# MoZhou1995/DeepPDE_ActorCritic

Measured on AMD Instinct MI355X. Metric: SDE trajectory-steps/sec (batch×horizon) at d=20; value-fn rel-L2 vs analytic, higher is better.
Workload: dtype f32

## Files before the change

### deeppde_actorcritic_amd/csrc/dpac_rollout_staged.h

```cpp
#pragma once

#ifndef DPAC_ST_CHUNKS
#define DPAC_ST_CHUNKS 4
#endif
#ifndef DPAC_ST_TIGHT
#define DPAC_ST_TIGHT 0
#endif
#ifndef DPAC_ST_TIGHT_CHUNKS
#define DPAC_ST_TIGHT_CHUNKS 3
#endif
#ifndef DPAC_ST_PREFETCH
#define DPAC_ST_PREFETCH 1
#endif
constexpr int kStCW = 4;
constexpr int kStCH = 16;
constexpr int kStPrefetch = DPAC_ST_PREFETCH;
static_assert(kStPrefetch == 0 || kStPrefetch == 1, "DPAC_ST_PREFETCH is 0 or 1");
template <typename T, int D, int P>
struct StagedPlan {
  static constexpr int TPW = kStCW * (64 / P);
  static constexpr int SLOT = TPW * D * (int)sizeof(T);
  static constexpr int PIECES = (SLOT + 1023) / 1024;
  static constexpr int kLdsCap = 128 * 1024;
  static constexpr int SLOT_1K = (SLOT + 16 + 1023) / 1024 * 1024;
  static constexpr int SLOT_16 = (SLOT + 16 + 15) / 16 * 16;
  static constexpr bool kWide = !DPAC_ST_TIGHT && DPAC_ST_CHUNKS * kStCH * SLOT_1K <= kLdsCap;
  static constexpr int CHUNKS = kWide ? DPAC_ST_CHUNKS : DPAC_ST_TIGHT_CHUNKS;
  static constexpr int SLOT_LDS = kWide ? SLOT_1K : SLOT_16;
  static constexpr int PADOFF = SLOT_LDS - 16;
  static constexpr int RS = CHUNKS * kStCH;
  static_assert(P < 4 || (SLOT % 16 == 0 && (PIECES - 1) * 1024 + 16 <= SLOT), "DMA pieces stay inside the slot");
  static constexpr bool kOk = P >= 4 && RS * SLOT_LDS <= kLdsCap && kStCH * PIECES <= 62;
};

template <class Fn, int... S>
__device__ __forceinline__ void unroll_phases(Fn& fn, std::integer_sequence<int, S...>) {
  (fn(Phase<S>{}), ...);
}

__device__ __forceinline__ int lds_load_relaxed(const int* p) {
  return __hip_atomic_load(p, __ATOMIC_RELAXED, __HIP_MEMORY_SCOPE_WORKGROUP);
}
__device__ __forceinline__ void lds_store_relaxed(int* p, int v) {
  __hip_atomic_store(p, v, __ATOMIC_RELAXED, __HIP_MEMORY_SCOPE_WORKGROUP);
}

template <int GEN>
constexpr int st_waves() { return kStCW + (GEN > 0 ? GEN : 1); }
#ifndef DPAC_ST_GEN
#define DPAC_ST_GEN 12
#endif
constexpr int kStGen = DPAC_ST_GEN;
static_assert(64 * st_waves<kStGen>() <= 1024, "DPAC_ST_GEN: a workgroup holds at most 1024 threads");

__device__ __forceinline__ void st_wait_consumed(const int* s_done, int need) {
  for (;;) {
    int mn = lds_load_relaxed(&s_done[0]);
#pragma unroll
    for (int w = 1; w < kStCW; ++w) mn = min(mn, lds_load_relaxed(&s_done[w]));
    if (mn >= need) break;
    __builtin_amdgcn_s_sleep(2);
  }
}
template <int NREADY>
__device__ __forceinline__ void st_wait_published(const int* s_ready, int want) {
  for (;;) {
    int mn = lds_load_relaxed(&s_ready[0]);
#pragma unroll
    for (int w = 1; w < NREADY; ++w) mn = min(mn, lds_load_relaxed(&s_ready[w]));
    if (mn >= want) break;
    __builtin_amdgcn_s_sleep(1);
  }
}

#ifndef DPAC_ST_TRACE
#define DPAC_ST_TRACE 0
#endif
#if DPAC_ST_TRACE
constexpr int kStTraceRow = 128, kStTraceWaves = 16, kStTraceChunks = 32;
static __device__ uint32_t g_st_trace[2 * kStTraceWaves * kStTraceRow];
__device__ __forceinline__ uint32_t st_clock() {
  unsigned long long t;
  __builtin_amdgcn_sched_barrier(0);
  asm volatile("s_memtime %0\n\ts_waitcnt lgkmcnt(0)" : "=s"(t)::"memory");
  __builtin_amdgcn_sched_barrier(0);
  return (uint32_t)t;
}
__device__ __forceinline__ uint32_t st_realtime() {
  unsigned long long t;
  __builtin_amdgcn_sched_barrier(0);
  asm volatile("s_memrealtime %0\n\ts_waitcnt lgkmcnt(0)" : "=s"(t)::"memory");
  __builtin_amdgcn_sched_barrier(0);
  return (uint32_t)t;
}
#define ST_PUT(pt, v)                \
  do {                               \
    const uint32_t st_v_ = (v);      \
    if (st_on) st_row[(pt)] = st_v_; \
  } while (0)
#define ST_MARK(pt) ST_PUT(pt, st_clock())
#define ST_CHUNK(base, c0) ((base) + ((c0) / kStCH < kStTraceChunks ? (c0) / kStCH : kStTraceChunks - 1))
#else
#define ST_PUT(pt, v) \
  do {                \
  } while (0)
#define ST_MARK(pt) \
  do {              \
  } while (0)
#endif

template <typename T, class E, int D, int SCHEME, int OUT, int GEN = 0>
__global__ __launch_bounds__(64 * st_waves<GEN>()) void k_rollout_staged(const E eq, const DevConsts<T> c,
                                                                          const RolloutArgs<T> a) {
  constexpr int P = E::kP, M = E::M, MC = E::MC;
  using PL = StagedPlan<T, D, P>;
  constexpr int TPW = PL::TPW, RS = PL::RS, PIECES = PL::PIECES, SLOT_LDS = PL::SLOT_LDS;
  constexpr bool COST = (OUT & kOutCost) != 0, WANT_U = (OUT & kOutU) != 0;
  constexpr int F = P < kStCH ? P : kStCH;
  constexpr int NREADY = GEN > 0 ? GEN : 1;
  static_assert(kStCH % F == 0 && (F & (F - 1)) == 0, "flush phase fixed per unrolled body");
  static_assert(GEN == 0 || (2 * M <= 4 && kStCH % 2 == 0), "generators draw the paired layout");
  using TR = Transition<T, E, SCHEME>;
  __shared__ __attribute__((aligned(16))) unsigned char s_ring[RS * SLOT_LDS];
  __shared__ int s_ready[NREADY], s_done[kStCW];
  const int wave = __builtin_amdgcn_readfirstlane((int)threadIdx.x / 64), lane = (int)threadIdx.x % 64;
  const int64_t row0 = xcd_block(blockIdx.x, gridDim.x) * TPW;
  const int N = a.N;
#if DPAC_ST_TRACE
  const bool st_on = lane == 0 && wave < kStTraceWaves && (blockIdx.x == 0 || blockIdx.x == gridDim.x - 1);
  uint32_t* const st_row = g_st_trace + ((blockIdx.x == 0 ? 0 : kStTraceWaves) + (wave < kStTraceWaves ? wave : 0)) * kStTraceRow;
  ST_MARK(0);
  ST_PUT(5, st_realtime());
#endif
  if (threadIdx.x == 0) {
#pragma unroll
    for (int w = 0; w < NREADY; ++w) s_ready[w] = 0;
#pragma unroll
    for (int w = 0; w < kStCW; ++w) s_done[w] = 0;
  }
  if (threadIdx.x < RS * 4)
    reinterpret_cast<uint32_t*>(s_ring + (threadIdx.x / 4) * SLOT_LDS + PL::PADOFF)[threadIdx.x % 4] = 0u;
  __syncthreads();
  ST_MARK(1);

  if constexpr (GEN > 0) {
    if (wave >= kStCW) {
      const int g = wave - kStCW;
      const int64_t rows_live = (a.B - row0) < TPW ? (a.B - row0) : TPW;
      constexpr int PLS = (D + M - 1) / M;
      constexpr int NBLK = (kStCH / 2) * TPW * PLS;
      constexpr int PASSES = (NBLK + 64 * GEN - 1) / (64 * GEN);
      constexpr int SLOT_T = SLOT_LDS / (int)sizeof(T);
      T* const ringw = reinterpret_cast<T*>(s_ring);
      for (int c0 = 0; c0 < N; c0 += kStCH) {
        const int need = c0 + kStCH - RS;
        if (need > 0) st_wait_consumed(s_done, need);
        asm volatile("" ::: "memory");
#pragma unroll 1
        for (int k = 0; k < PASSES; ++k) {
          const int e = (k * GEN + g) * 64 + lane;
          const int u = e / (TPW * PLS), rem = e - u * (TPW * PLS);
          const int i = rem / PLS, p = rem - i * PLS;
          const int t0 = c0 + 2 * u;
          if (e < NBLK && t0 < N && i < rows_live) {
            T v[4];
            dw_block_values<T>(a.seed, (uint64_t)(a.traj_offset + row0 + i), (uint64_t)(t0 >> 1) * P + p,
                               a.sample_type, v);
            T* d0 = ringw + (t0 % RS) * SLOT_T + i * D + p * M;
            T* d1 = ringw + ((t0 + 1) % RS) * SLOT_T + i * D + p * M;
#pragma unroll
            for (int m = 0; m < M; ++m) {
              if (p * M + m < D) {
                d0[m] = v[m];
                if (t0 + 1 < N) d1[m] = v[M + m];
              }
            }
          }
        }
        asm volatile("s_waitcnt lgkmcnt(0)" ::: "memory");
        if (lane == 0) lds_store_relaxed(&s_ready[g], c0 + kStCH < N ? c0 + kStCH : N);
      }
      return;
    }
  } else if (wave == kStCW) {
    const int64_t rows_live = (a.B - row0) < TPW ? (a.B - row0) : TPW;
    const uint32_t bytes = (uint32_t)(rows_live * D * (int64_t)sizeof(T));
    const uint32_t lds0 = (uint32_t)(uintptr_t)(__attribute__((address_space(3))) unsigned char*)s_ring;
    const char* base = (const char*)(a.dw + row0 * D);
    const int64_t step_bytes = a.B * D * (int64_t)sizeof(T);
    for (int c0 = 0; c0 < N; c0 += kStCH) {
      const int need = c0 + kStCH - RS;
      if (need > 0) st_wait_consumed(s_done, need);
      asm volatile("" ::: "memory");
#if DPAC_ST_TRACE
      ST_MARK(ST_CHUNK(16, c0));
#endif
#pragma unroll
      for (int s = 0; s < kStCH; ++s) {
        const int t = c0 + s < N ? c0 + s : N - 1;
        const char* src = base + t * step_bytes;
        const uint32_t slot = lds0 + (uint32_t)((t % RS) * SLOT_LDS);
#pragma unroll
        for (int k = 0; k < PIECES; ++k) {
          const uint32_t off = (uint32_t)((k * 64 + lane) * 16);
          const char* gp = src + (off < bytes ? off : 0u);
          const uint32_t m0 = __builtin_amdgcn_readfirstlane(slot + (uint32_t)(k * 1024));
          if (off < bytes || lane == 0) {
            int keep;
            asm volatile("s_mov_b32 %0, m0\n\ts_mov_b32 m0, %2\n\ts_nop 0\n\tglobal_load_lds_dwordx4 %1, off\n\ts_mov_b32 m0, %0"
                         : "=&s"(keep) : "v"(gp), "s"(m0) : "memory");
          }
        }
      }
#if DPAC_ST_TRACE
      ST_MARK(ST_CHUNK(48, c0));
#endif
      if (c0 > 0) {
        asm volatile("s_waitcnt vmcnt(%0)" ::"n"(kStCH * PIECES) : "memory");
        if (lane == 0) lds_store_relaxed(&s_ready[0], c0);
#if DPAC_ST_TRACE
        ST_MARK(ST_CHUNK(80, c0));
#endif
      }
    }
    asm volatile("s_waitcnt vmcnt(0)" ::: "memory");
    if (lane == 0) lds_store_relaxed(&s_ready[0], N);
    ST_MARK(4);
    ST_PUT(6, st_realtime());
    return;
  }

  const LaneCoord<P> lc(a.B, lane, row0 + wave * (64 / P));
  const int gl = wave * (64 / P) + lane / P;
  const Own<D, P> own(lc.p);
  const Own<E::CDIM, P> ownu(lc.p);
  const BufSlab<T, D, P> sx(own, lc.b, lc.live);
  const BufSlab<T, E::CDIM, P> su(ownu, lc.b, lc.live);
  const uint32_t slab = (uint32_t)(a.B * D * sizeof(T));
  const uint32_t slab_u = (uint32_t)(a.B * E::CDIM * sizeof(T));
  const uint32_t row_bytes = (uint32_t)(N * sizeof(T));
  const __amdgpu_buffer_rsrc_t rs_x = make_rsrc(a.x, slab * (uint32_t)(N + 1));
  const __amdgpu_buffer_rsrc_t rs_u = make_rsrc(a.u, WANT_U ? slab_u * (uint32_t)N : 0u);
  const __amdgpu_buffer_rsrc_t rs_dt = make_rsrc(a.dt, (uint32_t)a.B * row_bytes);
  const __amdgpu_buffer_rsrc_t rs_cf = make_rsrc(a.coef, (uint32_t)a.B * row_bytes);
  const T* ring = reinterpret_cast<const T*>(s_ring);
  const int lds_e = gl * D + lc.p * M;
  constexpr bool kVecRead = Own<D, P>::kFull && (M * sizeof(T) == 8 || M * sizeof(T) == 16);
  const uint32_t lane_off = own.active() ? (uint32_t)(lds_e * (int)sizeof(T)) : (uint32_t)PL::PADOFF;
  T keep = 0;
  auto flush = [&](int t_last, int count) {
    const uint32_t off = (lc.live && lc.p < count)
                             ? (uint32_t)((lc.b * N + t_last - lc.p) * (int64_t)sizeof(T)) : kOOB;
    buf_store_scalar<T>(rs_dt, off, fabs(keep));
    buf_store_scalar<T>(rs_cf, off, keep > T(0) ? T(1) : T(0));
  };
  T x[M];
  sx.load(make_rsrc(a.x0, slab), x);
  sx.store(rs_x, x);
  T r = TR::kRadius ? dsqrt(Lanes<P>::sum(sumsq(x))) : T(0);
  Flags fl = SCHEME == DPAC_SCHEME_ADAPTIVE ? region(r, c) : Flags{true, false};
  T disc = 1, y = 0;
  T xc[M], rc = r;
#pragma unroll
  for (int m = 0; m < M; ++m) xc[m] = x[m];
  T Ra = fl.alive ? c.R : -std::numeric_limits<T>::infinity();
  bool alive = fl.alive;
  const T sq0 = SCHEME == DPAC_SCHEME_ADAPTIVE ? dsqrt(c.dt0) : c.sqrt_dt0;
  T dt = c.dt0, sq = sq0;
  if constexpr (SCHEME == DPAC_SCHEME_ADAPTIVE) {
    dt = adaptive_dt_raw(fl.layer, r, c);
    dt = fl.layer ? fmax(dt, c.dt_min) : dt;
    sq = dsqrt(dt);
  }
  ST_MARK(2);
  auto read_dw_at = [&](int t, uint32_t slot_bytes, T (&dwv)[M]) {
    if constexpr (kVecRead) {
      typedef T vec __attribute__((ext_vector_type(M)));
      const vec v = *reinterpret_cast<const vec*>(s_ring + slot_bytes + lane_off);
#pragma unroll
      for (int m = 0; m < M; ++m) dwv[m] = v[m];
    } else {
      const T* slot = ring + (t % RS) * (SLOT_LDS / (int)sizeof(T)) + lds_e;
#pragma unroll
      for (int m = 0; m < M; ++m) dwv[m] = own.valid(m) ? slot[m] : T(0);
    }
  };
  auto read_dw = [&](int t, T (&dwv)[M]) { read_dw_at(t, (uint32_t)((t % RS) * SLOT_LDS), dwv); };
  auto step = [&](int t, const T (&dwv)[M], auto phase) {
    T uc[MC], f[M], s[M], xt[M];
    eq.u_true(xc, rc, uc);
    eq.drift(xc, uc, rc, f);
    eq.sigma(xc, uc, s);
#pragma unroll
    for (int m = 0; m < M; ++m) xt[m] = xc[m] + fma(f[m], dt, (s[m] * dwv[m]) * sq);
    const T St = Lanes<P>::sum(sumsq(xt));
    T u[MC];
    if constexpr (COST || WANT_U) eq.u_true(x, r, u);
    bool coef;
    T rt = T(0), dtn = dt, sqn = sq;
    if constexpr (SCHEME == DPAC_SCHEME_ADAPTIVE) {
      rt = dsqrt(St);
      const T b = Ra - rt;
      const bool inner = b - c.c_layer > T(0);
      coef = b > T(0);
      const T dtb = fmax((b * b) * c.inv_den, c.dt_min);
      const T sqb = dsqrt(dtb);
      const bool layer = coef && !inner;
      dtn = layer ? dtb : c.dt0;
      sqn = layer ? sqb : sq0;
      Ra = coef ? Ra : -std::numeric_limits<T>::infinity();
    } else {
      if constexpr (E::kNeedsNorm) rt = dsqrt(St);
      coef = alive && !(St - c.R2 >= T(0));
      alive = coef;
    }
    if constexpr (COST) {
      const T cf = coef ? T(1) : T(0);
      const T w = eq.w_finish(Lanes<P>::sum(eq.w_part(x, u)));
      y += cost_increment(a.cost_order, w, cf, dt, disc);
      disc = disc * disc_factor(dt, cf, c);
    }
    const T kv = coef ? dt : -dt;
#pragma unroll
    for (int m = 0; m < M; ++m) {
      x[m] = coef ? xt[m] : x[m];
      xc[m] = xt[m];
    }
    if constexpr (E::kNeedsNorm) {
      r = coef ? rt : r;
      rc = rt;
    }
    dt = dtn;
    sq = sqn;
    sx.template store<DPAC_ROLLOUT_X_AUX>(rs_x, x, (uint32_t)(t + 1) * slab);
    if constexpr (WANT_U) su.store(rs_u, u, (uint32_t)t * slab_u);
    constexpr int PH = decltype(phase)::value;
    keep = group_shift_in<P>(keep, kv, lc.p == 0);
    if constexpr (PH >= 0) {
      if constexpr (PH % F == F - 1) flush(t, F);
    } else if ((t & (F - 1)) == F - 1) {
      flush(t, F);
    }
  };
  constexpr bool kChunkRegs = kStPrefetch != 0 && !COST && GEN == 0;
  for (int c0 = 0; c0 < N; c0 += kStCH) {
    const int want = c0 + kStCH < N ? c0 + kStCH : N;
#if DPAC_ST_TRACE
    const uint32_t st_poll0 = st_clock();
#endif
    st_wait_published<NREADY>(s_ready, want);
    asm volatile("" ::: "memory");
#if DPAC_ST_TRACE
    {
      const uint32_t st_now = st_clock();
      ST_PUT(ST_CHUNK(16, c0), st_now);
      ST_PUT(ST_CHUNK(80, c0), st_now - st_poll0);
      if (c0 == 0) ST_PUT(3, st_now);
    }
#endif
    if constexpr (kChunkRegs) {
      auto steps = [&](int t0, auto count) {
        constexpr int CNT = decltype(count)::value;
        const uint32_t cb = (uint32_t)__builtin_amdgcn_readfirstlane((t0 % RS) * SLOT_LDS);
        T dwv[CNT][M];
#pragma unroll
        for (int q = 0; q < CNT; ++q) read_dw_at(t0 + q, cb + (uint32_t)(q * SLOT_LDS), dwv[q]);
        auto one = [&](auto sidx) {
          constexpr int S = decltype(sidx)::value;
          step(t0 + S, dwv[S], Phase<S>{});
        };
        unroll_phases(one, std::make_integer_sequence<int, CNT>{});
      };
      if (c0 + kStCH <= N) {
        steps(c0, Phase<kStCH>{});
      } else {
        static_assert(kStCH == 16, "remainder pieces of 8, 4, 2 and 1 steps");
        int t0 = c0;
        auto piece = [&](auto len) {
          if ((N - c0) & decltype(len)::value) {
            steps(t0, len);
            t0 += decltype(len)::value;
          }
        };
        piece(Phase<8>{});
        piece(Phase<4>{});
        piece(Phase<2>{});
        piece(Phase<1>{});
      }
    } else if (c0 + kStCH <= N) {
      const uint32_t cb = (uint32_t)__builtin_amdgcn_readfirstlane((c0 % RS) * SLOT_LDS);
      constexpr int PD = 1;
      T nxt[PD][M];
#pragma unroll
      for (int q = 0; q < PD; ++q) read_dw_at(c0 + q, cb + (uint32_t)(q * SLOT_LDS), nxt[q]);
      auto one = [&](auto sidx) {
        constexpr int S = decltype(sidx)::value;
        T cur[M];
#pragma unroll
        for (int m = 0; m < M; ++m) cur[m] = nxt[S % PD][m];
        if constexpr (S + PD < kStCH) read_dw_at(c0 + S + PD, cb + (uint32_t)((S + PD) * SLOT_LDS), nxt[S % PD]);
        step(c0 + S, cur, Phase<S>{});
      };
      unroll_phases(one, std::make_integer_sequence<int, kStCH>{});
    } else {
      for (int t = c0; t < N; ++t) {
        T cur[M];
        read_dw(t, cur);
        step(t, cur, Phase<-1>{});
      }
    }
    asm volatile("s_waitcnt lgkmcnt(0)" ::: "memory");
    if (lane == 0) lds_store_relaxed(&s_done[wave], want);
#if DPAC_ST_TRACE
    ST_MARK(ST_CHUNK(48, c0));
#endif
  }
  const int rem = N & (F - 1);
  if (rem) flush(N - 1, rem);
#if DPAC_ST_TRACE
  ST_MARK(4);
  asm volatile("s_waitcnt vmcnt(0)" ::: "memory");
  ST_MARK(7);
  ST_PUT(6, st_realtime());
#endif
  if constexpr (COST) {
    if (lc.live && lc.p == 0) {
      a.y[lc.b] = y;
      a.disc[lc.b] = disc;
    }
  }
}
```

Before: 28.18 billion.

## Preload first staged chunks of Brownian increments directly into registers

Compute waves now load the first HEAD chunks of dw (plus x0) straight from global memory into registers via buffer loads, and the DMA producer wave starts its LDS ring at step HS instead of zero. This removes the startup latency where compute waves wait for the producer to publish the first chunk, so the pipeline fill is overlapped with the initial steps. In exchange it costs extra VGPRs (capped by DPAC_ST_HEAD_VGPRS), which may lower occupancy, and adds select logic for remainder pieces inside the head chunks.

New measurement: 28.08 billion. About the same (-0.4%).

```diff
diff --git a/deeppde_actorcritic_amd/csrc/dpac_rollout_staged.h b/deeppde_actorcritic_amd/csrc/dpac_rollout_staged.h
--- a/deeppde_actorcritic_amd/csrc/dpac_rollout_staged.h
+++ b/deeppde_actorcritic_amd/csrc/dpac_rollout_staged.h
@@ -11,11 +11,24 @@
 #endif
 #ifndef DPAC_ST_PREFETCH
 #define DPAC_ST_PREFETCH 1
+#endif
+#ifndef DPAC_ST_HEAD
+#define DPAC_ST_HEAD 2
+#endif
+#ifndef DPAC_ST_HEAD_VGPRS
+#define DPAC_ST_HEAD_VGPRS 128
+#endif
+#ifndef DPAC_ST_HEAD_FENCE
+#define DPAC_ST_HEAD_FENCE 1
+#endif
+#ifndef DPAC_ST_HEAD_EARLY
+#define DPAC_ST_HEAD_EARLY 0
 #endif
 constexpr int kStCW = 4;
 constexpr int kStCH = 16;
 constexpr int kStPrefetch = DPAC_ST_PREFETCH;
 static_assert(kStPrefetch == 0 || kStPrefetch == 1, "DPAC_ST_PREFETCH is 0 or 1");
+static_assert(DPAC_ST_HEAD >= 0 && DPAC_ST_HEAD <= 4, "DPAC_ST_HEAD: 0 to 4 chunks");
 template <typename T, int D, int P>
 struct StagedPlan {
   static constexpr int TPW = kStCW * (64 / P);
@@ -31,6 +44,9 @@
   static constexpr int RS = CHUNKS * kStCH;
   static_assert(P < 4 || (SLOT % 16 == 0 && (PIECES - 1) * 1024 + 16 <= SLOT), "DMA pieces stay inside the slot");
   static constexpr bool kOk = P >= 4 && RS * SLOT_LDS <= kLdsCap && kStCH * PIECES <= 62;
+  static constexpr int kChunkDwords = kStCH * ((D + P - 1) / P) * (int)sizeof(T) / 4;
+  static constexpr int HEAD = DPAC_ST_HEAD * kChunkDwords <= DPAC_ST_HEAD_VGPRS ? DPAC_ST_HEAD
+                                                                               : DPAC_ST_HEAD_VGPRS / kChunkDwords;
 };
 
 template <class Fn, int... S>
@@ -109,6 +125,19 @@
   } while (0)
 #endif
 
+template <typename T, int D, int P, int HS>
+__device__ __forceinline__ void st_head_loads(const RolloutArgs<T>& a, int lane, int64_t group0,
+                                              T (&x)[Own<D, P>::M], T (&hd)[HS][Own<D, P>::M]) {
+  const LaneCoord<P> lc(a.B, lane, group0);
+  const BufSlab<T, D, P> sx(Own<D, P>(lc.p), lc.b, lc.live);
+  const uint32_t slab = (uint32_t)(a.B * D * sizeof(T));
+  sx.load(make_rsrc(a.x0, slab), x);
+  const __amdgpu_buffer_rsrc_t rs_dw = make_rsrc(a.dw, slab * (uint32_t)a.N);
+#pragma unroll
+  for (int q = 0; q < HS; ++q)
+    sx.template load<DPAC_ROLLOUT_DW_AUX>(rs_dw, hd[q], (uint32_t)(q < a.N ? q : a.N - 1) * slab);
+}
+
 template <typename T, class E, int D, int SCHEME, int OUT, int GEN = 0>
 __global__ __launch_bounds__(64 * st_waves<GEN>()) void k_rollout_staged(const E eq, const DevConsts<T> c,
                                                                           const RolloutArgs<T> a) {
@@ -120,6 +149,9 @@
   constexpr int NREADY = GEN > 0 ? GEN : 1;
   static_assert(kStCH % F == 0 && (F & (F - 1)) == 0, "flush phase fixed per unrolled body");
   static_assert(GEN == 0 || (2 * M <= 4 && kStCH % 2 == 0), "generators draw the paired layout");
+  constexpr bool kChunkRegs = kStPrefetch != 0 && !COST && GEN == 0;
+  constexpr int HS = kChunkRegs ? PL::HEAD * kStCH : 0;
+  constexpr bool kHeadEarly = DPAC_ST_HEAD_EARLY != 0;
   using TR = Transition<T, E, SCHEME>;
   __shared__ __attribute__((aligned(16))) unsigned char s_ring[RS * SLOT_LDS];
   __shared__ int s_ready[NREADY], s_done[kStCW];
@@ -132,6 +164,10 @@
   ST_MARK(0);
   ST_PUT(5, st_realtime());
 #endif
+  T x[M], hd[HS > 0 ? HS : 1][M];
+  if constexpr (HS > 0 && kHeadEarly) {
+    if (wave < kStCW) st_head_loads<T, D, P, HS>(a, lane, row0 + wave * (64 / P), x, hd);
+  }
   if (threadIdx.x == 0) {
 #pragma unroll
     for (int w = 0; w < NREADY; ++w) s_ready[w] = 0;
@@ -188,7 +224,7 @@
     const uint32_t lds0 = (uint32_t)(uintptr_t)(__attribute__((address_space(3))) unsigned char*)s_ring;
     const char* base = (const char*)(a.dw + row0 * D);
     const int64_t step_bytes = a.B * D * (int64_t)sizeof(T);
-    for (int c0 = 0; c0 < N; c0 += kStCH) {
+    for (int c0 = HS; c0 < N; c0 += kStCH) {
       const int need = c0 + kStCH - RS;
       if (need > 0) st_wait_consumed(s_done, need);
       asm volatile("" ::: "memory");
@@ -215,7 +251,7 @@
 #if DPAC_ST_TRACE
       ST_MARK(ST_CHUNK(48, c0));
 #endif
-      if (c0 > 0) {
+      if (c0 > HS) {
         asm volatile("s_waitcnt vmcnt(%0)" ::"n"(kStCH * PIECES) : "memory");
         if (lane == 0) lds_store_relaxed(&s_ready[0], c0);
 #if DPAC_ST_TRACE
@@ -254,8 +290,11 @@
     buf_store_scalar<T>(rs_dt, off, fabs(keep));
     buf_store_scalar<T>(rs_cf, off, keep > T(0) ? T(1) : T(0));
   };
-  T x[M];
-  sx.load(make_rsrc(a.x0, slab), x);
+  if constexpr (HS == 0) {
+    sx.load(make_rsrc(a.x0, slab), x);
+  } else if constexpr (!kHeadEarly) {
+    st_head_loads<T, D, P, HS>(a, lane, row0 + wave * (64 / P), x, hd);
+  }
   sx.store(rs_x, x);
   T r = TR::kRadius ? dsqrt(Lanes<P>::sum(sumsq(x))) : T(0);
   Flags fl = SCHEME == DPAC_SCHEME_ADAPTIVE ? region(r, c) : Flags{true, false};
@@ -342,43 +381,65 @@
       flush(t, F);
     }
   };
-  constexpr bool kChunkRegs = kStPrefetch != 0 && !COST && GEN == 0;
-  for (int c0 = 0; c0 < N; c0 += kStCH) {
-    const int want = c0 + kStCH < N ? c0 + kStCH : N;
-#if DPAC_ST_TRACE
-    const uint32_t st_poll0 = st_clock();
-#endif
-    st_wait_published<NREADY>(s_ready, want);
-    asm volatile("" ::: "memory");
-#if DPAC_ST_TRACE
-    {
-      const uint32_t st_now = st_clock();
-      ST_PUT(ST_CHUNK(16, c0), st_now);
-      ST_PUT(ST_CHUNK(80, c0), st_now - st_poll0);
-      if (c0 == 0) ST_PUT(3, st_now);
-    }
-#endif
-    if constexpr (kChunkRegs) {
-      auto steps = [&](int t0, auto count) {
-        constexpr int CNT = decltype(count)::value;
+  if constexpr (kChunkRegs) {
+    auto steps = [&](int t0, auto count, auto head) {
+      constexpr int CNT = decltype(count)::value, HC = decltype(head)::value;
+      T dwv[CNT][M];
+      if constexpr (HC >= 0) {
+        const int o = t0 - HC * kStCH;
+#pragma unroll
+        for (int q = 0; q < CNT; ++q) {
+#pragma unroll
+          for (int m = 0; m < M; ++m) {
+            T v = hd[HC * kStCH + q][m];
+#pragma unroll
+            for (int j = 1; j < kStCH / (2 * CNT); ++j) {
+              const T alt = hd[HC * kStCH + j * 2 * CNT + q][m];
+              v = o == j * 2 * CNT ? alt : v;
+            }
+            dwv[q][m] = v;
+          }
+        }
+      } else {
         const uint32_t cb = (uint32_t)__builtin_amdgcn_readfirstlane((t0 % RS) * SLOT_LDS);
-        T dwv[CNT][M];
 #pragma unroll
         for (int q = 0; q < CNT; ++q) read_dw_at(t0 + q, cb + (uint32_t)(q * SLOT_LDS), dwv[q]);
-        auto one = [&](auto sidx) {
-          constexpr int S = decltype(sidx)::value;
-          step(t0 + S, dwv[S], Phase<S>{});
-        };
-        unroll_phases(one, std::make_integer_sequence<int, CNT>{});
+      }
+      auto one = [&](auto sidx) {
+        constexpr int S = decltype(sidx)::value;
+        if constexpr (HC >= 0 && DPAC_ST_HEAD_FENCE > 0) {
+#pragma unroll
+          for (int m = 0; m < M; ++m) asm volatile("" : "+v"(dwv[S][m]));
+        }
+        step(t0 + S, dwv[S], Phase<S>{});
       };
+      unroll_phases(one, std::make_integer_sequence<int, CNT>{});
+    };
+    auto chunk = [&](int c0, auto head) {
+      const int want = c0 + kStCH < N ? c0 + kStCH : N;
+#if DPAC_ST_TRACE
+      const uint32_t st_poll0 = st_clock();
+#endif
+      if constexpr (decltype(head)::value < 0) {
+        st_wait_published<NREADY>(s_ready, want);
+        asm volatile("" ::: "memory");
+      }
+#if DPAC_ST_TRACE
+      {
+        const uint32_t st_now = st_clock();
+        ST_PUT(ST_CHUNK(16, c0), st_now);
+        ST_PUT(ST_CHUNK(80, c0), st_now - st_poll0);
+        if (c0 == 0) ST_PUT(3, st_now);
+      }
+#endif
       if (c0 + kStCH <= N) {
-        steps(c0, Phase<kStCH>{});
+        steps(c0, Phase<kStCH>{}, head);
       } else {
         static_assert(kStCH == 16, "remainder pieces of 8, 4, 2 and 1 steps");
         int t0 = c0;
         auto piece = [&](auto len) {
           if ((N - c0) & decltype(len)::value) {
-            steps(t0, len);
+            steps(t0, len, head);
             t0 += decltype(len)::value;
           }
         };
@@ -386,34 +447,71 @@
         piece(Phase<4>{});
         piece(Phase<2>{});
         piece(Phase<1>{});
-      }
-    } else if (c0 + kStCH <= N) {
-      const uint32_t cb = (uint32_t)__builtin_amdgcn_readfirstlane((c0 % RS) * SLOT_LDS);
-      constexpr int PD = 1;
-      T nxt[PD][M];
-#pragma unroll
-      for (int q = 0; q < PD; ++q) read_dw_at(c0 + q, cb + (uint32_t)(q * SLOT_LDS), nxt[q]);
-      auto one = [&](auto sidx) {
-        constexpr int S = decltype(sidx)::value;
-        T cur[M];
-#pragma unroll
-        for (int m = 0; m < M; ++m) cur[m] = nxt[S % PD][m];
-        if constexpr (S + PD < kStCH) read_dw_at(c0 + S + PD, cb + (uint32_t)((S + PD) * SLOT_LDS), nxt[S % PD]);
-        step(c0 + S, cur, Phase<S>{});
-      };
-      unroll_phases(one, std::make_integer_sequence<int, kStCH>{});
-    } else {
-      for (int t = c0; t < N; ++t) {
-        T cur[M];
-        read_dw(t, cur);
-        step(t, cur, Phase<-1>{});
-      }
-    }
-    asm volatile("s_waitcnt lgkmcnt(0)" ::: "memory");
-    if (lane == 0) lds_store_relaxed(&s_done[wave], want);
-#if DPAC_ST_TRACE
-    ST_MARK(ST_CHUNK(48, c0));
-#endif
+        if constexpr (decltype(head)::value >= 0) {
+          const T last = hd[HS - 1][M - 1];
+          asm volatile("" ::"v"(last));
+        }
+      }
+      asm volatile("s_waitcnt lgkmcnt(0)" ::: "memory");
+      if (lane == 0) lds_store_relaxed(&s_done[wave], want);
+#if DPAC_ST_TRACE
+      ST_MARK(ST_CHUNK(48, c0));
+#endif
+    };
+    auto head_chunk = [&](auto h) {
+      if (decltype(h)::value * kStCH < N) {
+        chunk(decltype(h)::value * kStCH, h);
+      } else {
+        const T last = hd[HS - 1][M - 1];
+        asm volatile("" ::"v"(last));
+      }
+    };
+    unroll_phases(head_chunk, std::make_integer_sequence<int, HS / kStCH>{});
+    for (int c0 = HS; c0 < N; c0 += kStCH) chunk(c0, Phase<-1>{});
+  } else {
+    for (int c0 = 0; c0 < N; c0 += kStCH) {
+      const int want = c0 + kStCH < N ? c0 + kStCH : N;
+#if DPAC_ST_TRACE
+      const uint32_t st_poll0 = st_clock();
+#endif
+      st_wait_published<NREADY>(s_ready, want);
+      asm volatile("" ::: "memory");
+#if DPAC_ST_TRACE
+      {
+        const uint32_t st_now = st_clock();
+        ST_PUT(ST_CHUNK(16, c0), st_now);
+        ST_PUT(ST_CHUNK(80, c0), st_now - st_poll0);
+        if (c0 == 0) ST_PUT(3, st_now);
+      }
+#endif
+      if (c0 + kStCH <= N) {
+        const uint32_t cb = (uint32_t)__builtin_amdgcn_readfirstlane((c0 % RS) * SLOT_LDS);
+        constexpr int PD = 1;
+        T nxt[PD][M];
+#pragma unroll
+        for (int q = 0; q < PD; ++q) read_dw_at(c0 + q, cb + (uint32_t)(q * SLOT_LDS), nxt[q]);
+        auto one = [&](auto sidx) {
+          constexpr int S = decltype(sidx)::value;
+          T cur[M];
+#pragma unroll
+          for (int m = 0; m < M; ++m) cur[m] = nxt[S % PD][m];
+          if constexpr (S + PD < kStCH) read_dw_at(c0 + S + PD, cb + (uint32_t)((S + PD) * SLOT_LDS), nxt[S % PD]);
+          step(c0 + S, cur, Phase<S>{});
+        };
+        unroll_phases(one, std::make_integer_sequence<int, kStCH>{});
+      } else {
+        for (int t = c0; t < N; ++t) {
+          T cur[M];
+          read_dw(t, cur);
+          step(t, cur, Phase<-1>{});
+        }
+      }
+      asm volatile("s_waitcnt lgkmcnt(0)" ::: "memory");
+      if (lane == 0) lds_store_relaxed(&s_done[wave], want);
+#if DPAC_ST_TRACE
+      ST_MARK(ST_CHUNK(48, c0));
+#endif
+    }
   }
   const int rem = N & (F - 1);
   if (rem) flush(N - 1, rem);
```
